# apache/datafusion-comet

Hardware: NVIDIA H100
Metric: rows/sec on TPC-H Q1 filter+agg (higher is better)
Workload: dtype i128

## Files before the change

datafusion-comet_b200/csrc/abi.cpp:

```cpp
#include "../../include/comet_b200.h"

#include "abi_internal.h"
#include "parquet_kernels.h"
#include "exec_internal.h"
#include "jit.h"
#include "plan.h"
#include "proto_wire.h"

#include <cstring>
#include <functional>
#include <map>
#include <mutex>

using namespace cb200;

namespace {

struct CtxRes {
    cudaStream_t stream;
    int* d_err;
    int* h_err;
    cudaEvent_t ev0, ev1;
};
std::mutex g_pool_mu;
std::map<int, std::vector<CtxRes>> g_pool;

void parse_config(const uint8_t* cfg, size_t len, ExecContext& ctx) {
    if (!cfg || !len) return;
    PbReader r(cfg, len);
    while (r.next()) {
        if (r.field != 1 || r.wire != 2) { r.skip(); continue; }
        PbReader e = r.sub();
        std::string k, v;
        while (e.next()) {
            if (e.field == 1) k = e.bytes();
            else if (e.field == 2) v = e.bytes();
            else e.skip();
        }
        if (k == "spark.comet.b200.chunkRows") ctx.chunk_rows = std::max<int64_t>(1024, atoll(v.c_str()));
        else if (k == "spark.comet.batchSize") ctx.batch_size = atoi(v.c_str());
        else if (k == "spark.comet.b200.streamAgg.minRows") ctx.stream_agg_min_rows = atoll(v.c_str());
        else if (k == "spark.comet.b200.streamAgg.maxRatio") ctx.stream_agg_max_ratio = atof(v.c_str());
        else if (k == "spark.comet.b200.hashThreads") { int t = atoi(v.c_str()); if (t == 256 || t == 512 || t == 768 || t == 960) ctx.hash_threads = t; }
    }
}
// ... 5 lines not shown
    cuda_check(cudaSetDevice(ctx.device), "cudaSetDevice");
    {
        struct DevInfo { int major = 0, minor = 0, sms = 0; bool known = false; };
        static DevInfo info[64];
        static std::mutex info_mu;
        std::lock_guard<std::mutex> lk(info_mu);
        if (ctx.device < 0 || ctx.device >= 64) throw ExecError(CB200_ERR_CUDA, "", "device ordinal out of range");
        DevInfo& di = info[ctx.device];
        if (!di.known) {
            cuda_check(cudaDeviceGetAttribute(&di.major, cudaDevAttrComputeCapabilityMajor, ctx.device), "cudaDeviceGetAttribute");
            cuda_check(cudaDeviceGetAttribute(&di.minor, cudaDevAttrComputeCapabilityMinor, ctx.device), "cudaDeviceGetAttribute");
            cuda_check(cudaDeviceGetAttribute(&di.sms, cudaDevAttrMultiProcessorCount, ctx.device), "cudaDeviceGetAttribute");
            di.known = true;
        }
        if (di.major != 9 || di.minor != 0) throw ExecError(CB200_ERR_CUDA, "", "comet_b200 kernels are built for sm_90a; device is sm_" + std::to_string(di.major * 10 + di.minor));
        ctx.num_sms = di.sms;
    }
    {
        std::lock_guard<std::mutex> lk(g_pool_mu);
        auto& fl = g_pool[ctx.device];
        if (!fl.empty()) {
            CtxRes r = fl.back();
            fl.pop_back();
            ctx.stream = r.stream; ctx.d_err = r.d_err; ctx.h_err = r.h_err; ctx.ev0 = r.ev0; ctx.ev1 = r.ev1;
        }
    }
    if (!ctx.stream) {
        cuda_check(cudaStreamCreateWithFlags(&ctx.stream, cudaStreamNonBlocking), "cudaStreamCreate");
        cudaMemPool_t pool;
        if (cudaDeviceGetDefaultMemPool(&pool, ctx.device) == cudaSuccess) {
            unsigned long long keep = ~0ull;
            cudaMemPoolSetAttribute(pool, cudaMemPoolAttrReleaseThreshold, &keep);
        }
        cuda_check(cudaMalloc((void**)&ctx.d_err, 64), "cudaMalloc err");
        cuda_check(cudaMallocHost((void**)&ctx.h_err, 64), "cudaMallocHost err");
        cuda_check(cudaEventCreate(&ctx.ev0), "cudaEventCreate");
        cuda_check(cudaEventCreate(&ctx.ev1), "cudaEventCreate");
    }
    cuda_check(cudaMemsetAsync(ctx.d_err, 0, 64, ctx.stream), "memset err");
    set_alloc_stream(ctx.stream);
    p->root = build_exec(p->op, &ctx, &p->inputs);
    p->started = true;
}

DType dtype_from_ids(int type_id, int precision, int scale) {
    if (type_id < 0 || type_id > 13) throw Unsupported("type id " + std::to_string(type_id));
    DType d;
    d.id = (TypeId)type_id;
    d.precision = precision;
    d.scale = scale;
    return d;
}

}

extern "C" {

const char* cb200_version(void) { return "comet_b200 0.1.0 (sm_90a; reference apache/datafusion-comet 1.1.0 @2699f59b)"; }

int cb200_supports(const uint8_t* op_proto, size_t op_len, cb200_error* why) {
// ... 83 lines not shown
                o.host_values = c.h_data.data();
                o.host_validity_bytes = c.h_valid.empty() ? nullptr : c.h_valid.data();
            } else {
                o.values = c.data ? c.data->ptr : nullptr;
                o.validity = c.validity ? c.validity->ptr : nullptr;
                o.validity_bytes = c.valid_bytes ? c.valid_bytes->ptr : nullptr;
                o.bool_bytes = c.bool_bytes ? c.bool_bytes->ptr : nullptr;
                if (c.is_dict) { o.n_dict = (int)c.dict->values().size(); o.value_width = phys_bytes(c.phys); }
            }
        }
    });
}

void cb200_release(cb200_plan* plan) {
    if (!plan) return;
    TraceSpan ts("release");
    try {
        if (plan->started) cudaSetDevice(plan->ctx.device);
        plan->last = Batch();
        plan->root.reset();
        if (plan->ctx.stream) {
            cudaStreamSynchronize(plan->ctx.stream);
            std::lock_guard<std::mutex> lk(g_pool_mu);
            g_pool[plan->ctx.device].push_back(CtxRes{plan->ctx.stream, plan->ctx.d_err, plan->ctx.h_err, plan->ctx.ev0, plan->ctx.ev1});
        }
        for (auto* s : plan->inputs.streams) if (s && s->release) s->release(s);
    } catch (...) {
    }
    delete plan;
}

cb200_table* cb200_table_create(int64_t n_rows) {
    auto* t = new cb200_table();
    t->t = std::make_shared<DeviceTable>();
    t->t->n_rows = n_rows;
    return t;
}

int cb200_table_add_column(cb200_table* t, int32_t type_id, int32_t precision, int32_t scale, int32_t value_width, const void* dev_values,
                           const void* dev_validity, int64_t null_count, const char* const* dict_values, int32_t n_dict, cb200_error* err) {
    return cb200_guarded(err, [&]() -> int {
        if (!t) throw PlanError("null table handle");
        Column c;
        c.type = dtype_from_ids(type_id, precision, scale);
        size_t n = (size_t)t->t->n_rows;
        if (n_dict > 0) {
            if (!c.type.is_string()) throw PlanError("dictionary values on a non-string column");
// ... 205 lines not shown
```

datafusion-comet_b200/csrc/agg.cpp:

```cpp
#include "exec_internal.h"
#include "../../include/comet_b200.h"

#include "aot_kernels.h"
#include "ranges.h"

#include <algorithm>
#include <mutex>

namespace cb200 {

static std::mutex g_profile_mu;
static std::map<std::string, std::vector<int>> g_range_profile;

void reset_range_profiles() {
    std::lock_guard<std::mutex> lk(g_profile_mu);
    g_range_profile.clear();
}

namespace {

enum class Strategy { Undecided, Dense, Table, Stream };
enum Level { SAFE = 0, TYPE = 1, TIGHT = 2 };
constexpr int DENSE_MAX_GROUPS = 64;

constexpr int GK = CB_GID_RANGES;
struct HashFlags { int w[CB_HFLAG_WORDS]; };
int64_t round_ids(int64_t n) { return (n + GK - 1) / GK * GK; }

using ValueMasks = uint64_t[CB_MAX_COLS * 2];
// ... 2 lines not shown

std::vector<int> decode_gid(int g, const std::vector<int>& cards) {
    std::vector<int> code(cards.size());
    for (int k = (int)cards.size() - 1; k >= 0; k--) { code[(size_t)k] = g % cards[(size_t)k]; g /= cards[(size_t)k]; }
    return code;
}

int grid_for(const ExecContext* ctx, int n_tiles) { return std::max(1, std::min(ctx->num_sms, n_tiles)); }

struct Kernel {
    PipelineSpec spec;
    GeneratedKernel g;
    std::shared_ptr<CompiledModule> mod;
};

void launch_named(ExecContext* ctx, const Kernel& k, const char* name, dim3 grid, dim3 block, void** args) {
    cuda_check(cudaLaunchKernel((const void*)k.mod->kernel(name), grid, block, args, 0, ctx->stream), name);
    ctx->kernel_launches++;
}

struct DenseState {
    std::vector<int> cards;
    std::vector<bool> has_null;
    DeviceBufP totals, spill, partials;
    int groups = 0;

    void regroup(ExecContext* ctx, int n_words, const std::vector<int>& word_kinds, const std::vector<int>& new_cards) {
        int new_groups = 1;
        for (int c : new_cards) new_groups *= c;
        std::vector<uint64_t> oldt((size_t)groups * n_words * 2), newt((size_t)new_groups * n_words * 2);
        cuda_check(cudaMemcpy(oldt.data(), totals->ptr, oldt.size() * 8, cudaMemcpyDeviceToHost), "regroup D2H");
        for (size_t i = 0; i < (size_t)new_groups * n_words; i++) newt[i * 2] = identity_word(word_kinds[i % (size_t)n_words]);
        for (int g = 0; g < groups; g++) {
            const std::vector<int> code = decode_gid(g, cards);
            int ng = 0, mul = 1;
            for (int k = (int)cards.size() - 1; k >= 0; k--) {
                int cd = code[(size_t)k];
                if (has_null[(size_t)k] && cd == cards[(size_t)k] - 1) cd = new_cards[(size_t)k] - 1;
                ng += cd * mul;
                mul *= new_cards[(size_t)k];
            }
            memcpy(&newt[(size_t)ng * n_words * 2], &oldt[(size_t)g * n_words * 2], (size_t)n_words * 16);
        }
        totals = host_to_device(newt.data(), newt.size() * 8, ctx, "regroup H2D");
        groups = new_groups;
    }

// ... 385 lines not shown
    }

    void clear_vmask() {
        if (!vmask) vmask = std::make_shared<DeviceBuf>(CB_MAX_COLS * 16);
        cuda_check(cudaMemsetAsync(vmask->ptr, 0, CB_MAX_COLS * 16, ctx->stream), "memset vmask");
    }
    void copy_vmask(ValueMasks& masks) {
        cuda_check(cudaMemcpyAsync(masks, vmask->ptr, sizeof(ValueMasks), cudaMemcpyDeviceToHost, ctx->stream), "read value masks"); ctx->d2h_bytes += (int64_t)(sizeof(ValueMasks));
    }
    static std::vector<int> mask_bits(const PipelineSpec& spec, const ValueMasks& masks) {
        std::vector<int> seen(spec.cols.size(), -1);
        for (size_t i = 0; i < spec.cols.size(); i++) {
            if (!spec.cols[i].type.is_decimal()) continue;
            uint64_t lo = masks[2 * i], hi = masks[2 * i + 1];
            seen[i] = hi ? 64 + r_bitlen(hi) : r_bitlen(lo);
        }
        return seen;
    }
    void observe(const std::vector<int>& seen) {
        for (size_t i = 0; i < seen.size(); i++)
            if (seen[i] >= 0) observed_bits[(size_t)used_cols[i]] = std::max(observed_bits[(size_t)used_cols[i]], seen[i]);
    }

    int prepare_key(Batch& b, size_t k) {
        int ci = keys[k]->index;
        Column& c = b.cols[ci];
        if (c.type.id == TypeId::Bool) return 2;
        if (!c.type.is_string()) return -1;
        if (c.is_dict) {
            key_dicts[k] = c.dict;
            return (int)c.dict->values().size();
        }
        if (!dev_dicts[k]) {
            auto dd = std::make_shared<DevDict>();
            const int64_t cap = 1 << 16;
            const int max_codes = 4096;
            const int64_t bytes_cap = 1 << 20;
            auto alloc = [&](size_t n) { auto bfr = std::make_shared<DeviceBuf>(n); cuda_check(cudaMemsetAsync(bfr->ptr, 0, bfr->bytes, ctx->stream), "memset dict"); dd->bufs.push_back(bfr); return bfr->ptr; };
            dd->d.tags = (unsigned long long*)alloc((size_t)cap * 8);
            dd->d.slot_code = (int*)alloc((size_t)cap * 4);
            dd->d.capacity = cap;
            dd->d.n_codes = (int*)alloc(64);
            dd->d.bytes_used = (unsigned long long*)((char*)dd->d.n_codes + 16);
            dd->d.err = (int*)((char*)dd->d.n_codes + 32);
            dd->d.max_codes = max_codes;
            dd->d.code_off = (long long*)alloc((size_t)max_codes * 8);
            dd->d.code_len = (int*)alloc((size_t)max_codes * 4);
            dd->d.bytes = (unsigned char*)alloc((size_t)bytes_cap);
            dd->d.bytes_cap = bytes_cap;
            dev_dicts[k] = dd;
            key_dicts[k] = std::make_shared<Dictionary>();
        }
        DevDict& dd = *dev_dicts[k];
        if (!c.offsets || !c.chars) throw Unsupported("string key column without offsets/chars buffers");
        auto row_slot = std::make_shared<DeviceBuf>((size_t)b.n_rows * 4);
        auto codes = std::make_shared<DeviceBuf>((size_t)b.n_rows * 4);
        launch_dict_encode(dd.d, (const int*)c.offsets->ptr, (const unsigned char*)c.chars->ptr, c.validity ? (const unsigned char*)c.validity->ptr : nullptr,
                           b.n_rows, (int*)row_slot->ptr, (int*)codes->ptr, ctx->stream);
        ctx->kernel_launches += 2;
        int hdr[12];
        cuda_check(cudaMemcpyAsync(hdr, dd.d.n_codes, sizeof(hdr), cudaMemcpyDeviceToHost, ctx->stream), "dict header");
        cuda_check(cudaStreamSynchronize(ctx->stream), "dict encode");
        int n_codes = hdr[0], derr = hdr[8];
        if (derr & CB_DICT_FULL) throw Unsupported("plain Utf8 group key with more distinct values than the device dictionary holds (dictionary-encode the column)");
        if (derr & CB_DICT_COLLISION) throw ExecError(14, "", "64-bit hash collision between distinct group key strings");
        if (n_codes > dd.host_known) {
            std::vector<long long> off((size_t)n_codes);
            std::vector<int> len((size_t)n_codes);
            cuda_check(cudaMemcpy(off.data(), dd.d.code_off, (size_t)n_codes * 8, cudaMemcpyDeviceToHost), "dict offsets");
            cuda_check(cudaMemcpy(len.data(), dd.d.code_len, (size_t)n_codes * 4, cudaMemcpyDeviceToHost), "dict lengths");
            for (int i = dd.host_known; i < n_codes; i++) {
                std::string s((size_t)len[(size_t)i], '\0');
                if (len[(size_t)i]) cuda_check(cudaMemcpy(&s[0], dd.d.bytes + off[(size_t)i], (size_t)len[(size_t)i], cudaMemcpyDeviceToHost), "dict bytes");
                key_dicts[k]->append(s);
            }
            dd.host_known = n_codes;
        }
        c.data = codes;
        c.phys = Phys::I32;
        c.is_dict = true;
        c.dict = key_dicts[k];
        return n_codes;
    }

    void consume(Batch& b) {
        for (int ci : used_cols) if (b.cols[(size_t)ci].validity) col_nullable[(size_t)ci] = true;
        std::vector<int> nc(keys.size());
        std::vector<bool> hn(keys.size());
        for (size_t k = 0; k < keys.size(); k++) {
            int card = prepare_key(b, k);
            const Column& c = b.cols[keys[k]->index];
            hn[k] = key_has_null[k] || c.validity != nullptr;
            nc[k] = card < 0 ? -1 : std::max(card, 1) + (hn[k] ? 1 : 0);
            if (!dense.cards.empty() && nc[k] >= 0) nc[k] = std::max(nc[k], dense.cards[k]);
        }
        bool densifiable = true;
        for (int c : nc) if (c < 0) densifiable = false;
// ... 41 lines not shown
            run_range(b, SAMPLE, b.n_rows, n_groups, TIGHT);
        } else {
            run_range(b, 0, b.n_rows, n_groups, have_obs ? TIGHT : TYPE);
        }
        if (!profile_key.empty()) {
            std::lock_guard<std::mutex> lk(g_profile_mu);
            if (g_range_profile.size() > 256) g_range_profile.clear();
            g_range_profile[profile_key] = observed_bits;
        }
    }

    void leave_dense() {
        if (mode == AggMode::Final) throw Unsupported("group cardinality grew past the dense path mid-stream in a Final aggregate");
        if (have_totals()) {
            Batch early;
            dense.finalize(ctx, last, certified_params(), ungrouped, schema, key_dicts, early);
            if (early.n_rows > 0) outq.push_back(std::move(early));
        }
        last = Kernel();
        dense = DenseState();
        n_words = 0; word_kinds.clear(); role_words.clear(); rows_scanned = 0;
    }

    void run_range(Batch& b, int64_t row0, int64_t row1, int n_groups, Level lv) {
        TraceSpan tsr("agg.run_range");
        while (true) {
            Kernel k;
            {
                TraceSpan ts("agg.codegen+jit");
                k = compile(make_spec(&b, Strategy::Dense, n_groups, lv));
            }
            const int64_t max_rows = (int64_t)ctx->num_sms * k.g.threads * (1ll << CB_RPT_LOG2) / 1024 * 1024;
            int64_t r0 = row0;
            while (r0 < row1 && launch_one(b, r0, std::min(row1, r0 + max_rows), n_groups, k, lv)) r0 += max_rows;
            if (r0 >= row1) return;
            if (lv == SAFE) throw ExecError(15, "", "internal: value-mask validation failed without assumptions");
            lv = lv == TIGHT ? TYPE : SAFE;
            row0 = r0;
        }
    }

    bool launch_one(Batch& b, int64_t r0, int64_t r1, int n_groups, const Kernel& k, Level lv) {
        cudaStream_t st = ctx->stream;
        size_t tot_bytes = (size_t)n_groups * n_words * 16;
        if (!have_totals()) {
            dense.totals = std::make_shared<DeviceBuf>(tot_bytes);
            dense.groups = n_groups;
        }
        if (!dense.spill || dense.spill->bytes < tot_bytes) {
            dense.spill = std::make_shared<DeviceBuf>(tot_bytes);
            cuda_check(cudaMemsetAsync(dense.spill->ptr, 0, dense.spill->bytes, st), "memset spill");
        }
        clear_vmask();
        cb::PipeParams p;
        fill_inputs(p, b, k.g.tile, r0, r1);
        bind_str_masks(p, k.spec, b);
        int grid = grid_for(ctx, p.n_tiles);
        size_t part_bytes = (size_t)grid * tot_bytes;
        if (!dense.partials || dense.partials->bytes < part_bytes) dense.partials = std::make_shared<DeviceBuf>(part_bytes);
        p.n_groups = n_groups;
        for (size_t i = 0; i < dense.cards.size() && i < CB_MAX_KEYS; i++) p.key_card[i] = dense.cards[i];
        p.partials = (cb::u8*)dense.partials->ptr;
        p.spill = (cb::u64*)dense.spill->ptr;
        p.vmask = (cb::u64*)vmask->ptr;
        launch(k.mod->kernel(k.g.entry), dim3(grid), dim3(k.g.threads + 32), k.g.dyn_smem(n_groups), &p);
        ctx->pipeline_rows += r1 - r0;
        ValueMasks masks;
        copy_vmask(masks);
        const int errs = ctx->take_device_errors();
        const std::vector<int> seen = mask_bits(k.spec, masks);
        bool ok = true;
        for (size_t i = 0; i < seen.size(); i++)
            if (k.spec.cols[i].assume_bits > 0 && seen[i] > k.spec.cols[i].assume_bits) ok = false;
        observe(seen);
        if (!ok) {
            cuda_check(cudaMemsetAsync(dense.spill->ptr, 0, dense.spill->bytes, st), "memset spill");
            ctx->agg_range_reruns++;
            return false;
        }
        ctx->raise_device_errors(errs);
        ctx->agg_range_levels |= lv == TIGHT ? CB200_RANGE_TIGHT : lv == TYPE ? CB200_RANGE_TYPE : CB200_RANGE_SAFE;
        rows_scanned += r1 - r0;
        cb::FinParams fp;
        memset(&fp, 0, sizeof(fp));
        fp.partials = (const cb::u64*)dense.partials->ptr;
        fp.spill = (cb::u64*)dense.spill->ptr;
        fp.totals = (cb::u64*)dense.totals->ptr;
        fp.n_ctas = grid;
        fp.n_groups = n_groups;
        fp.first = have_totals() ? 0 : 1;
        fp.err = ctx->d_err;
        int total_words = n_groups * n_words;
        void* args[] = {&fp};
        cuda_check(cudaLaunchKernel((const void*)k.mod->kernel("cb_fold"), dim3((total_words + 127) / 128), dim3(128), args, 0, st), "fold launch");
        ctx->kernel_launches++;
        last = k;
        return true;
    }

    void launch_id_rows(Batch& b, int64_t r0, int64_t r1, const Kernel& k, bool with_table) {
        clear_vmask();
        cb::PipeParams p;
        fill_inputs(p, b, k.g.tile, r0, r1);
        bind_str_masks(p, k.spec, b);
        p.hkeys = with_table ? (cb::u64*)table.hkeys->ptr : nullptr;
        p.hkey_of_gid = (cb::u64*)rows.hkey_of_gid->ptr;
        p.htotals = (cb::u64*)rows.htotals->ptr;
        p.hmask = with_table ? (cb::u32)(table.hcap - 1) : 0;
        p.max_groups = (cb::i32)rows.max_groups;
        p.hflags = (cb::i32*)rows.hflags->ptr;
        p.vmask = (cb::u64*)vmask->ptr;
        p.n_groups = 2;
        launch(k.mod->kernel(k.g.entry), dim3(grid_for(ctx, p.n_tiles)), dim3(k.g.threads + 32), k.g.dyn_smem(0), &p);
    }

    void consume_table(Batch& b) {
        const Kernel k = compile(make_spec(&b, Strategy::Table, 2, SAFE));
        {
            TraceSpan ts("hash.ensure_table");
            table.ensure(ctx, k, rows, b.n_rows, child->rows_hint(), rows_scanned, mode != AggMode::Partial || !all_partial);
// ... 88 lines not shown
            fp.cert_b[ai][1] = b >= RSAT ? ~0ull : (uint64_t)(b >> 64);
            const bool direct = aggs[ai].mode != AggMode::Partial || aggs[ai].children[0]->kind == ExprKind::Bound;
            if (b < RSAT && b != 0 && direct) fp.cert_b[ai][1] |= 1ull << 63;
        }
        return fp;
    }

    bool next(Batch& out) override {
        if (!emitted) aggregate_input();
        if (outq_pos >= outq.size()) return false;
        out = std::move(outq[outq_pos++]);
        return true;
    }
    void aggregate_input() {
        if (keys.size() > CB_MAX_KEYS) throw Unsupported("more than 4 group keys");
        key_has_null.assign(keys.size(), false);
        col_nullable.assign(child->schema.size(), false);
        key_dicts.assign(keys.size(), nullptr);
        dev_dicts.assign(keys.size(), nullptr);
        Batch in;
        while (child->next(in)) {
            if (in.n_rows == 0) continue;
            consume(in);
            ctx->check_device_errors();
        }
        emitted = true;
        if (!have_totals()) {
            if (!ungrouped) return;
            last = compile(make_spec(nullptr, Strategy::Dense, 1));
            std::vector<uint64_t> id((size_t)n_words * 2, 0);
            for (int w = 0; w < n_words; w++) id[(size_t)w * 2] = identity_word(word_kinds[(size_t)w]);
            dense.totals = std::make_shared<DeviceBuf>(id.size() * 8);
            cuda_check(cudaMemcpyAsync(dense.totals->ptr, id.data(), id.size() * 8, cudaMemcpyHostToDevice, ctx->stream), "identity totals");
            cuda_check(cudaStreamSynchronize(ctx->stream), "identity totals sync");
            dense.groups = 1;
        }
        Batch result;
        if (strategy == Strategy::Table || strategy == Strategy::Stream) rows.finalize(ctx, last, certified_params(), key_dicts, result);
        else dense.finalize(ctx, last, certified_params(), ungrouped, schema, key_dicts, result);
        outq.push_back(std::move(result));
    }
};

}

ExecNodeP make_agg_node(const OperatorP& agg_op, const ExecNodeP& src, const std::vector<ExprP>& preds, const std::vector<ExprP>& cols, ExecContext* ctx,
                        const std::vector<int>& assume_bits) {
// ... 54 lines not shown
```

datafusion-comet_b200/csrc/exec.cpp:

```cpp
#include "exec_internal.h"

#include <cstdlib>
#include <ctime>
#include <mutex>

namespace cb200 {

enum { ERR_I128_OVERFLOW = 0, ERR_ANSI_OVERFLOW = 1, ERR_ORDER_DEPENDENT = 2, ERR_DIVIDE_BY_ZERO = 3, ERR_ARROW_DIVIDE_BY_ZERO = 4, ERR_DICT_CODE = 5,
       ERR_WIDE_MINMAX = 6 };

bool trace_on() {
    static int on = -1;
    if (on < 0) { const char* e = getenv("CB200_TRACE"); on = (e && *e && *e != '0') ? 1 : 0; }
    return on == 1;
}
double now_ms() {
    struct timespec ts;
    clock_gettime(CLOCK_MONOTONIC, &ts);
    return ts.tv_sec * 1e3 + ts.tv_nsec * 1e-6;
}
TraceSpan::TraceSpan(const char* n) : name(n), t0(trace_on() ? now_ms() : 0) {}
TraceSpan::~TraceSpan() {
    if (trace_on()) { static const double tz = now_ms(); const double t1 = now_ms(); fprintf(stderr, "[cb200 trace] %-28s %8.3f ms   (ends at +%.3f ms)\n", name, t1 - t0, t1 - tz); }
}
// ... 68 lines not shown
        cudaStreamSynchronize(stream);
        e = cudaMallocAsync(&ptr, bytes, stream);
    }
    cuda_check(e, "cudaMallocAsync");
}
DeviceBuf::~DeviceBuf() {
    if (!(owned && ptr)) return;
    if (bytes >= BLOCK_CACHE_MIN && bytes == size_class(bytes)) {
        BlockCache& c = g_block_cache[current_device()];
        cudaEvent_t ev = nullptr;
        if (cudaEventCreateWithFlags(&ev, cudaEventDisableTiming) == cudaSuccess && cudaEventRecord(ev, stream) == cudaSuccess) {
            std::lock_guard<std::mutex> lk(c.mu);
            if (c.cached_bytes + bytes <= block_cache_limit()) {
                c.free_blocks.insert({bytes, CachedBlock{ptr, stream, ev}});
                c.cached_bytes += bytes;
                return;
            }
        }
        if (ev) cudaEventDestroy(ev);
    }
    cudaFreeAsync(ptr, stream);
}

void ExecContext::collect_timing() {
    if (!ev_pending) return;
    float ms = 0;
    if (cudaEventElapsedTime(&ms, ev0, ev1) == cudaSuccess) { pipeline_ms += ms; pipeline_launches++; }
    ev_pending = false;
}

int ExecContext::take_device_errors() {
    cuda_check(cudaMemcpyAsync(h_err, d_err, sizeof(int), cudaMemcpyDeviceToHost, stream), "error flag copy");
    cuda_check(cudaStreamSynchronize(stream), "stream sync");
    collect_timing();
    int e = *h_err;
    if (e) cudaMemsetAsync(d_err, 0, sizeof(int), stream);
    return e;
}

void ExecContext::raise_device_errors(int e) {
    if (!e) return;
    if (e & (1 << ERR_ANSI_OVERFLOW))
        throw ExecError(10, "ARITHMETIC_OVERFLOW", "[ARITHMETIC_OVERFLOW] overflow in ANSI mode");
    if (e & (1 << ERR_DIVIDE_BY_ZERO))
        throw ExecError(10, "DIVIDE_BY_ZERO", "[DIVIDE_BY_ZERO] Division by zero. Use `try_divide` to tolerate divisor being 0 and return NULL instead. "
                                              "If necessary set \"spark.sql.ansi.enabled\" to \"false\" to bypass this error.");
    if (e & (1 << ERR_ARROW_DIVIDE_BY_ZERO)) throw ExecError(11, "", "Arrow error: Divide by zero error");
    if (e & (1 << ERR_I128_OVERFLOW))
        throw ExecError(11, "", "Arrow error: Arithmetic overflow: Overflow happened on decimal arithmetic");
    if (e & (1 << ERR_DICT_CODE))
        throw ExecError(3, "", "dictionary code out of range: a non-NULL row of a dictionary-encoded string column has a code outside its dictionary");
// ... 164 lines not shown
        std::vector<ArrowArray> arrs;
        int64_t total = 0;
        while (total < ctx->chunk_rows) {
            ArrowArray a;
            memset(&a, 0, sizeof(a));
            if (stream->get_next(stream, &a) != 0) {
                const char* m = stream->get_last_error ? stream->get_last_error(stream) : nullptr;
                for (auto& x : arrs) if (x.release) x.release(&x);
                throw ExecError(3, "", std::string("ArrowArrayStream get_next failed: ") + (m ? m : "?"));
            }
            if (!a.release) { eof = true; break; }
            if (a.length > 0) { total += a.length; arrs.push_back(a); }
            else a.release(&a);
        }
        if (arrs.empty()) return false;
        try {
            upload(arrs, total, out);
        } catch (...) {
            for (auto& x : arrs) if (x.release) x.release(&x);
            throw;
        }
        cuda_check(cudaStreamSynchronize(ctx->stream), "H2D copies");
        for (auto& x : arrs) if (x.release) x.release(&x);
        return true;
    }

    std::vector<int32_t> unify_dict(size_t col, const ArrowArray* d) {
        Dictionary& g = *dicts[col];
        const int32_t* off = (const int32_t*)d->buffers[1] + d->offset;
        const char* chars = (const char*)d->buffers[2];
        std::vector<int32_t> remap((size_t)d->length);
        bool identity = true;
        for (int64_t k = 0; k < d->length; k++) {
            const int32_t code = g.intern(std::string(chars + off[k], (size_t)(off[k + 1] - off[k])));
            remap[(size_t)k] = code;
            if (code != k) identity = false;
        }
        if (identity) remap.clear();
        return remap;
    }

    cudaError_t h2d(void* dst, const void* src, size_t n) {
        ctx->h2d_bytes += (int64_t)n;
        return cudaMemcpyAsync(dst, src, n, cudaMemcpyHostToDevice, ctx->stream);
    }

    void upload(std::vector<ArrowArray>& arrs, int64_t total, Batch& out) {
        TraceSpan ts("source.upload");
        out.n_rows = total;
        out.cols.clear();
        out.cols.resize(schema.size());
        cudaStream_t st = ctx->stream;
        for (size_t c = 0; c < schema.size(); c++) {
            Column& col = out.cols[c];
            col.type = schema[c];
            bool any_nulls = false;
            for (auto& a : arrs) {
                ArrowArray* ch = a.children[c];
                if (ch->null_count != 0 && ch->buffers[0]) any_nulls = true;
            }
            if (any_nulls) {
                col.validity = std::make_shared<DeviceBuf>((size_t)(total + 7) / 8 + 8);
                cuda_check(cudaMemsetAsync(col.validity->ptr, 0, col.validity->bytes, st), "memset validity");
            }
            std::vector<DeviceBufP> temps;
            if (col_is_dict[c]) {
                col.is_dict = true;
                col.dict = dicts[c];
                int w = dict_index_width[c];
                bool need_remap = false;
                std::vector<std::vector<int32_t>> remaps;
                for (auto& a : arrs) {
                    remaps.push_back(unify_dict(c, a.children[c]->dictionary));
                    if (!remaps.back().empty()) need_remap = true;
                }
                if (!need_remap) {
                    col.phys = w == 1 ? Phys::I8 : w == 2 ? Phys::I16 : Phys::I32;
                    col.data = std::make_shared<DeviceBuf>((size_t)total * w);
                } else {
                    col.phys = Phys::I32;
                    col.data = std::make_shared<DeviceBuf>((size_t)total * 4);
                }
                int64_t row = 0;
                for (size_t k = 0; k < arrs.size(); k++) {
                    ArrowArray* ch = arrs[k].children[c];
                    const char* src = (const char*)ch->buffers[1] + ch->offset * w;
                    if (!need_remap) {
                        cuda_check(h2d((char*)col.data->ptr + row * w, src, (size_t)ch->length * w), "H2D dict codes");
                    } else {
                        auto tmp = std::make_shared<DeviceBuf>((size_t)ch->length * w);
                        temps.push_back(tmp);
                        cuda_check(h2d(tmp->ptr, src, (size_t)ch->length * w), "H2D dict codes");
                        std::vector<int32_t> table = remaps[k];
                        if (table.empty()) { table.resize((size_t)ch->dictionary->length); for (size_t i = 0; i < table.size(); i++) table[i] = (int32_t)i; }
                        DeviceBufP dt = host_to_device(table.data(), table.size() * 4, ctx, "H2D remap table");
                        ctx->h2d_bytes += (int64_t)(table.size() * 4);
                        temps.push_back(dt);
                        launch_remap_codes(tmp->ptr, w, ch->length, (const int*)dt->ptr, (int)table.size(), (int*)col.data->ptr + row, st);
                    }
                    row += ch->length;
                }
            } else if (schema[c].is_string()) {
                int64_t total_chars = 0;
                for (auto& a : arrs) {
                    ArrowArray* ch = a.children[c];
                    const int32_t* off = (const int32_t*)ch->buffers[1] + ch->offset;
                    total_chars += off[ch->length] - off[0];
                }
                if (total_chars > INT32_MAX) throw Unsupported("more than 2 GiB of string data in one chunk");
                col.chars = std::make_shared<DeviceBuf>((size_t)total_chars + 16);
                std::vector<int32_t> offs((size_t)total + 1);
                int64_t row = 0;
                int32_t base = 0;
                for (auto& a : arrs) {
                    ArrowArray* ch = a.children[c];
                    const int32_t* off = (const int32_t*)ch->buffers[1] + ch->offset;
                    for (int64_t i = 0; i < ch->length; i++) offs[(size_t)(row + i)] = base + (off[i] - off[0]);
                    int32_t nchars = off[ch->length] - off[0];
                    if (nchars) cuda_check(h2d((char*)col.chars->ptr + base, (const char*)ch->buffers[2] + off[0], (size_t)nchars), "H2D chars");
                    base += nchars;
                    row += ch->length;
                }
                offs[(size_t)total] = base;
                col.offsets = host_to_device(offs.data(), offs.size() * 4, ctx, "H2D offsets");
                ctx->h2d_bytes += (int64_t)(offs.size() * 4);
                col.phys = Phys::I32;
            } else {
                col.phys = phys_of(schema[c]);
                int w = schema[c].arrow_width();
                if (w == 0) {
                    col.data = std::make_shared<DeviceBuf>((size_t)(total + 7) / 8 + 8);
                    cuda_check(cudaMemsetAsync(col.data->ptr, 0, col.data->bytes, st), "memset bool");
                    int64_t row = 0;
                    for (auto& a : arrs) {
                        ArrowArray* ch = a.children[c];
                        append_bits((uint32_t*)col.data->ptr, row, (const uint8_t*)ch->buffers[1], ch->offset, ch->length, temps);
                        row += ch->length;
                    }
                } else {
                    col.data = std::make_shared<DeviceBuf>((size_t)total * w);
                    int64_t row = 0;
                    for (auto& a : arrs) {
                        ArrowArray* ch = a.children[c];
                        cuda_check(h2d((char*)col.data->ptr + row * w, (const char*)ch->buffers[1] + ch->offset * w, (size_t)ch->length * w), "H2D column");
                        row += ch->length;
                    }
                }
            }
            if (any_nulls) {
                int64_t row = 0, nulls = 0;
                for (auto& a : arrs) {
                    ArrowArray* ch = a.children[c];
                    bool has = ch->null_count != 0 && ch->buffers[0];
                    append_bits((uint32_t*)col.validity->ptr, row, has ? (const uint8_t*)ch->buffers[0] : nullptr, ch->offset, ch->length, temps);
                    nulls += has ? (ch->null_count < 0 ? 1 : ch->null_count) : 0;
                    row += ch->length;
                }
                col.null_count = nulls;
            }
            if (!temps.empty()) cuda_check(cudaStreamSynchronize(st), "temp buffers");
        }
    }

    void append_bits(uint32_t* dst, int64_t row, const uint8_t* src, int64_t src_off, int64_t n, std::vector<DeviceBufP>& temps) {
        if (n <= 0) return;
        if (src && (row & 7) == 0 && (src_off & 7) == 0 && ((n & 7) == 0)) {
            cuda_check(h2d((char*)dst + (row >> 3), src + (src_off >> 3), (size_t)(n >> 3)), "H2D bitmap");
            return;
        }
        const uint8_t* dsrc = nullptr;
        int64_t doff = 0;
        if (src) {
            int64_t b0 = src_off >> 3, b1 = (src_off + n + 7) >> 3;
            auto tmp = std::make_shared<DeviceBuf>((size_t)(b1 - b0) + 8);
            temps.push_back(tmp);
            cuda_check(h2d(tmp->ptr, src + b0, (size_t)(b1 - b0)), "H2D bitmap");
            dsrc = (const uint8_t*)tmp->ptr;
            doff = src_off & 7;
        }
        launch_bitmap_append(dst, row, dsrc, doff, n, ctx->stream);
    }
};

// ... 459 lines not shown
```

datafusion-comet_b200/csrc/exec.h:

```cpp
#pragma once
#include "arrow_abi.h"
#include "codegen.h"
#include "jit.h"
#include "plan.h"

#include <cuda_runtime.h>
#include <climits>
#include <memory>
#include <string>
#include <unordered_map>
#include <vector>

namespace cb200 {

struct ExecError : std::runtime_error {
    int code;
    std::string error_class;
    ExecError(int c, const std::string& cls, const std::string& msg) : std::runtime_error(msg), code(c), error_class(cls) {}
};

void cuda_check(cudaError_t e, const char* what);

struct TraceSpan {
    const char* name;
// ... 62 lines not shown
    bool on_host = false;
    std::vector<uint8_t> h_data;
    std::vector<uint8_t> h_valid;
    std::vector<int32_t> h_offsets;
};

struct Batch {
    int64_t n_rows = 0;
    std::vector<Column> cols;
};

struct ExecContext {
    int device = 0;
    cudaStream_t stream = nullptr;
    int num_sms = 132;
    int64_t chunk_rows = 1ll << 26;
    int hash_threads = 512;
    int64_t stream_agg_min_rows = 4 << 20;
    double stream_agg_max_ratio = 0.5;
    int batch_size = 8192;
    int* d_err = nullptr;
    int* h_err = nullptr;
    int64_t kernel_launches = 0;
    cudaEvent_t ev0 = nullptr, ev1 = nullptr;
    bool ev_pending = false;
    double pipeline_ms = 0;
    int64_t pipeline_launches = 0;
    int64_t pipeline_rows = 0;
    int64_t h2d_bytes = 0, d2h_bytes = 0;
    int64_t scan_pruned_row_groups = 0, scan_pruned_rows = 0;
    int64_t scan_pruned_pages = 0, scan_page_pruned_rows = 0;
    int64_t agg_strategies = 0;
    int64_t agg_range_levels = 0;
    int64_t agg_range_reruns = 0;
    int64_t sort_rows = 0, sort_passes = 0, sort_pass_rows = 0;
    int64_t sort_select_rows = 0;
    int64_t join_build_rows = 0, join_probe_rows = 0, join_out_rows = 0;
    int64_t join_cond_pairs = 0;
    double partition_ids_ms = 0, partition_place_ms = 0, partition_gather_ms = 0;
    std::vector<int64_t> partition_starts;
    void check_device_errors() { raise_device_errors(take_device_errors()); }
    int take_device_errors();
    void raise_device_errors(int e);
    void collect_timing();
};

struct ExecNode {
    std::vector<DType> schema;
// ... 33 lines not shown
```

datafusion-comet_b200/csrc/exec_internal.h:

```cpp
#pragma once
#include "exec.h"

#include "aot_kernels.h"
#include "device/cb_params.h"

#include <algorithm>
#include <cstring>
#include <functional>
#include <map>
#include <set>

namespace cb200 {

static constexpr size_t SMEM_BUDGET = 220 * 1024;

inline Phys phys_of(const DType& t) {
    switch (t.id) {
    case TypeId::Bool: return Phys::Bitmap;
    case TypeId::Int8: return Phys::I8;
    case TypeId::Int16: return Phys::I16;
    case TypeId::Int32: case TypeId::Date: return Phys::I32;
    case TypeId::Int64: case TypeId::Timestamp: case TypeId::TimestampNtz: return Phys::I64;
    case TypeId::Float32: return Phys::F32;
    case TypeId::Float64: return Phys::F64;
// ... 89 lines not shown
            rewrite_bound(c, slot_of);
            out.push_back(c);
        }
        return out;
    }
    void fill_inputs(cb::PipeParams& p, const Batch& b, int tile, int64_t row0 = 0, int64_t row1 = -1) const { fill_inputs_of(p, b, used_cols, tile, row0, row1); }
    void fill_inputs_of(cb::PipeParams& p, const Batch& b, const std::vector<int>& which, int tile, int64_t row0 = 0, int64_t row1 = -1) const {
        memset(&p, 0, sizeof(p));
        if (row1 < 0) row1 = b.n_rows;
        if (row0 & 1023) throw ExecError(15, "", "internal: launch range must start on a 1024-row boundary");
        for (size_t i = 0; i < which.size(); i++) {
            const Column& c = b.cols[which[i]];
            if (!c.data) throw Unsupported("column " + std::to_string(which[i]) + " (" + c.type.str() + ") has no fixed-width device representation");
            int w = phys_bytes(c.phys);
            p.col[i] = (const cb::u8*)c.data->ptr + (w == 0 ? row0 / 8 : row0 * w);
            p.val[i] = c.validity ? (const cb::u8*)c.validity->ptr + row0 / 8 : nullptr;
        }
        p.n_rows = row1 - row0;
        p.n_tiles = (int)((p.n_rows + tile - 1) / tile);
        p.err = ctx->d_err;
    }
    StrMasks str_masks;
    void bind_str_masks(cb::PipeParams& p, const PipelineSpec& spec, const Batch& b) { str_masks.bind(p, spec, b, ctx); }
    void launch(cudaKernel_t k, dim3 grid, dim3 block, size_t smem, void* params) {
        cuda_check(cudaFuncSetAttribute((const void*)k, cudaFuncAttributeMaxDynamicSharedMemorySize, (int)smem), "cudaFuncSetAttribute(smem)");
        void* args[] = {params};
        if (ctx->ev_pending) { cuda_check(cudaStreamSynchronize(ctx->stream), "stream sync"); ctx->collect_timing(); }
        cuda_check(cudaEventRecord(ctx->ev0, ctx->stream), "event record");
        cuda_check(cudaLaunchKernel((const void*)k, grid, block, args, smem, ctx->stream), "kernel launch");
        cuda_check(cudaEventRecord(ctx->ev1, ctx->stream), "event record");
        ctx->ev_pending = true;
        ctx->kernel_launches++;
    }
};

PipelineSpec count_pass_spec(std::vector<SourceCol> cols, std::vector<ExprP> predicates);

ExecNodeP make_agg_node(const OperatorP& agg_op, const ExecNodeP& src, const std::vector<ExprP>& preds, const std::vector<ExprP>& cols, ExecContext* ctx,
                        const std::vector<int>& assume_bits);
ExecNodeP make_partition_node(const OperatorP& op, const ExecNodeP& child, ExecContext* ctx);
ExecNodeP make_sort_node(const OperatorP& op, const ExecNodeP& child, ExecContext* ctx);
ExecNodeP make_join_node(const OperatorP& op, const ExecNodeP& left, const ExecNodeP& right, ExecContext* ctx);

int key_kind(const Column& c);
DeviceBufP host_to_device(const void* p, size_t n, ExecContext* ctx, const char* what);
void columns_to_device(Batch& b, ExecContext* ctx);
void arrive(Batch& b, ExecContext* ctx, const char* op);
Batch drain(ExecNode& child, ExecContext* ctx, const char* op, const char* concat_op);
template <typename I> void gather_columns(const Batch& in, const I* row_idx, int64_t n, Batch& out, ExecContext* ctx, const char* op);
void gather_columns_or_null(const Batch& in, const unsigned* row_idx, int64_t n, Batch& out, ExecContext* ctx);
Batch concat_batches(const std::vector<Batch>& bs, ExecContext* ctx, const char* op);
cb::SortKeyCol key_field(const Column& c, bool has_null, int& off);
struct RowKeys { DeviceBufP keys; uint64_t and_or[2 * cb::SK_MAX_WORDS]; std::vector<int> digits; };
RowKeys pack_row_keys(const cb::SortKeyCols& kc, int64_t n, int bits, ExecContext* ctx);
// ... 10 lines not shown
```

Before: 38.87 billion.

## Batch dense-agg sub-range launches and defer host syncs and validation readback

The dense aggregation path now launches all sub-range pipeline kernels back to back, each with its own partials/spill slot and value-mask scratch, then does a single D2H readback and stream sync before validating and folding. Previously every sub-range did its own launch, vmask copy and sync. Several other syncs go too: the per-column temp-buffer sync during upload (host vectors are kept alive until the batch sync instead), the per-batch device error check, and the per-string copies when decoding the string dictionary, which now uses one prefetch copy. Timing events become a growable per-launch array. The cost is more device memory for per-slot buffers, plus more complex rerun logic that recurses into fresh slots.

```diff
diff --git a/datafusion-comet_b200/csrc/abi.cpp b/datafusion-comet_b200/csrc/abi.cpp
--- a/datafusion-comet_b200/csrc/abi.cpp
+++ b/datafusion-comet_b200/csrc/abi.cpp
@@ -20,7 +20,7 @@
     cudaStream_t stream;
     int* d_err;
     int* h_err;
-    cudaEvent_t ev0, ev1;
+    std::vector<cudaEvent_t> ev;
 };
 std::mutex g_pool_mu;
 std::map<int, std::vector<CtxRes>> g_pool;
@@ -72,7 +72,7 @@
         if (!fl.empty()) {
             CtxRes r = fl.back();
             fl.pop_back();
-            ctx.stream = r.stream; ctx.d_err = r.d_err; ctx.h_err = r.h_err; ctx.ev0 = r.ev0; ctx.ev1 = r.ev1;
+            ctx.stream = r.stream; ctx.d_err = r.d_err; ctx.h_err = r.h_err; ctx.ev = r.ev;
         }
     }
     if (!ctx.stream) {
@@ -84,8 +84,6 @@
         }
         cuda_check(cudaMalloc((void**)&ctx.d_err, 64), "cudaMalloc err");
         cuda_check(cudaMallocHost((void**)&ctx.h_err, 64), "cudaMallocHost err");
-        cuda_check(cudaEventCreate(&ctx.ev0), "cudaEventCreate");
-        cuda_check(cudaEventCreate(&ctx.ev1), "cudaEventCreate");
     }
     cuda_check(cudaMemsetAsync(ctx.d_err, 0, 64, ctx.stream), "memset err");
     set_alloc_stream(ctx.stream);
@@ -215,7 +213,7 @@
         if (plan->ctx.stream) {
             cudaStreamSynchronize(plan->ctx.stream);
             std::lock_guard<std::mutex> lk(g_pool_mu);
-            g_pool[plan->ctx.device].push_back(CtxRes{plan->ctx.stream, plan->ctx.d_err, plan->ctx.h_err, plan->ctx.ev0, plan->ctx.ev1});
+            g_pool[plan->ctx.device].push_back(CtxRes{plan->ctx.stream, plan->ctx.d_err, plan->ctx.h_err, plan->ctx.ev});
         }
         for (auto* s : plan->inputs.streams) if (s && s->release) s->release(s);
     } catch (...) {
diff --git a/datafusion-comet_b200/csrc/agg.cpp b/datafusion-comet_b200/csrc/agg.cpp
--- a/datafusion-comet_b200/csrc/agg.cpp
+++ b/datafusion-comet_b200/csrc/agg.cpp
@@ -5,6 +5,7 @@
 #include "ranges.h"
 
 #include <algorithm>
+#include <climits>
 #include <mutex>
 
 namespace cb200 {
@@ -53,7 +54,7 @@
 struct DenseState {
     std::vector<int> cards;
     std::vector<bool> has_null;
-    DeviceBufP totals, spill, partials;
+    DeviceBufP totals;
     int groups = 0;
 
     void regroup(ExecContext* ctx, int n_words, const std::vector<int>& word_kinds, const std::vector<int>& new_cards) {
@@ -485,6 +486,7 @@
             if (seen[i] >= 0) observed_bits[(size_t)used_cols[i]] = std::max(observed_bits[(size_t)used_cols[i]], seen[i]);
     }
 
+    static constexpr size_t DICT_PREFETCH = 1 << 16;
     int prepare_key(Batch& b, size_t k) {
         int ci = keys[k]->index;
         Column& c = b.cols[ci];
@@ -499,7 +501,14 @@
             const int64_t cap = 1 << 16;
             const int max_codes = 4096;
             const int64_t bytes_cap = 1 << 20;
-            auto alloc = [&](size_t n) { auto bfr = std::make_shared<DeviceBuf>(n); cuda_check(cudaMemsetAsync(bfr->ptr, 0, bfr->bytes, ctx->stream), "memset dict"); dd->bufs.push_back(bfr); return bfr->ptr; };
+            const size_t sizes[] = {(size_t)cap * 8, (size_t)cap * 4, 64, (size_t)max_codes * 8, (size_t)max_codes * 4, (size_t)bytes_cap};
+            size_t total = 0;
+            for (size_t s : sizes) total += (s + 255) / 256 * 256;
+            auto whole = std::make_shared<DeviceBuf>(total);
+            cuda_check(cudaMemsetAsync(whole->ptr, 0, whole->bytes, ctx->stream), "memset dict");
+            dd->bufs.push_back(whole);
+            size_t at = 0;
+            auto alloc = [&](size_t n) { void* q = (char*)whole->ptr + at; at += (n + 255) / 256 * 256; return q; };
             dd->d.tags = (unsigned long long*)alloc((size_t)cap * 8);
             dd->d.slot_code = (int*)alloc((size_t)cap * 4);
             dd->d.capacity = cap;
@@ -521,21 +530,31 @@
         launch_dict_encode(dd.d, (const int*)c.offsets->ptr, (const unsigned char*)c.chars->ptr, c.validity ? (const unsigned char*)c.validity->ptr : nullptr,
                            b.n_rows, (int*)row_slot->ptr, (int*)codes->ptr, ctx->stream);
         ctx->kernel_launches += 2;
+        const char* head = (const char*)dd.d.n_codes;
+        const size_t o_off = (size_t)((const char*)dd.d.code_off - head), o_len = (size_t)((const char*)dd.d.code_len - head);
+        const size_t o_bytes = (size_t)((const char*)dd.d.bytes - head);
+        std::unique_ptr<char[]> h(new char[o_bytes + DICT_PREFETCH]);
+        cuda_check(cudaMemcpyAsync(h.get(), head, o_bytes + DICT_PREFETCH, cudaMemcpyDeviceToHost, ctx->stream), "dict header");
+        cuda_check(cudaStreamSynchronize(ctx->stream), "dict encode");
         int hdr[12];
-        cuda_check(cudaMemcpyAsync(hdr, dd.d.n_codes, sizeof(hdr), cudaMemcpyDeviceToHost, ctx->stream), "dict header");
-        cuda_check(cudaStreamSynchronize(ctx->stream), "dict encode");
+        memcpy(hdr, h.get(), sizeof(hdr));
         int n_codes = hdr[0], derr = hdr[8];
         if (derr & CB_DICT_FULL) throw Unsupported("plain Utf8 group key with more distinct values than the device dictionary holds (dictionary-encode the column)");
         if (derr & CB_DICT_COLLISION) throw ExecError(14, "", "64-bit hash collision between distinct group key strings");
         if (n_codes > dd.host_known) {
-            std::vector<long long> off((size_t)n_codes);
-            std::vector<int> len((size_t)n_codes);
-            cuda_check(cudaMemcpy(off.data(), dd.d.code_off, (size_t)n_codes * 8, cudaMemcpyDeviceToHost), "dict offsets");
-            cuda_check(cudaMemcpy(len.data(), dd.d.code_len, (size_t)n_codes * 4, cudaMemcpyDeviceToHost), "dict lengths");
+            const long long* off = (const long long*)(h.get() + o_off);
+            const int* len = (const int*)(h.get() + o_len);
+            long long lo = LLONG_MAX, hi = 0;
+            for (int i = dd.host_known; i < n_codes; i++) { lo = std::min(lo, off[i]); hi = std::max(hi, off[i] + len[i]); }
+            const char* bytes = h.get() + o_bytes;
+            std::vector<char> more;
+            if (hi > (long long)DICT_PREFETCH) {
+                more.resize((size_t)(hi - lo));
+                cuda_check(cudaMemcpy(more.data(), dd.d.bytes + lo, more.size(), cudaMemcpyDeviceToHost), "dict bytes");
+            }
             for (int i = dd.host_known; i < n_codes; i++) {
-                std::string s((size_t)len[(size_t)i], '\0');
-                if (len[(size_t)i]) cuda_check(cudaMemcpy(&s[0], dd.d.bytes + off[(size_t)i], (size_t)len[(size_t)i], cudaMemcpyDeviceToHost), "dict bytes");
-                key_dicts[k]->append(s);
+                const char* sp = more.empty() ? bytes + off[i] : more.data() + (off[i] - lo);
+                key_dicts[k]->append(std::string(sp, (size_t)len[i]));
             }
             dd.host_known = n_codes;
         }
@@ -623,80 +642,96 @@
         n_words = 0; word_kinds.clear(); role_words.clear(); rows_scanned = 0;
     }
 
-    void run_range(Batch& b, int64_t row0, int64_t row1, int n_groups, Level lv) {
+    void run_range(Batch& b, int64_t row0, int64_t row1, int n_groups, Level lv, size_t slot0 = 0) {
         TraceSpan tsr("agg.run_range");
-        while (true) {
-            Kernel k;
-            {
-                TraceSpan ts("agg.codegen+jit");
-                k = compile(make_spec(&b, Strategy::Dense, n_groups, lv));
-            }
-            const int64_t max_rows = (int64_t)ctx->num_sms * k.g.threads * (1ll << CB_RPT_LOG2) / 1024 * 1024;
-            int64_t r0 = row0;
-            while (r0 < row1 && launch_one(b, r0, std::min(row1, r0 + max_rows), n_groups, k, lv)) r0 += max_rows;
-            if (r0 >= row1) return;
-            if (lv == SAFE) throw ExecError(15, "", "internal: value-mask validation failed without assumptions");
-            lv = lv == TIGHT ? TYPE : SAFE;
-            row0 = r0;
-        }
-    }
-
-    bool launch_one(Batch& b, int64_t r0, int64_t r1, int n_groups, const Kernel& k, Level lv) {
-        cudaStream_t st = ctx->stream;
-        size_t tot_bytes = (size_t)n_groups * n_words * 16;
+        Kernel k;
+        {
+            TraceSpan ts("agg.codegen+jit");
+            k = compile(make_spec(&b, Strategy::Dense, n_groups, lv));
+        }
+        const int64_t max_rows = (int64_t)ctx->num_sms * k.g.threads * (1ll << CB_RPT_LOG2) / 1024 * 1024;
+        const size_t tot_bytes = (size_t)n_groups * n_words * 16;
         if (!have_totals()) {
             dense.totals = std::make_shared<DeviceBuf>(tot_bytes);
             dense.groups = n_groups;
         }
-        if (!dense.spill || dense.spill->bytes < tot_bytes) {
-            dense.spill = std::make_shared<DeviceBuf>(tot_bytes);
-            cuda_check(cudaMemsetAsync(dense.spill->ptr, 0, dense.spill->bytes, st), "memset spill");
-        }
-        clear_vmask();
-        cb::PipeParams p;
-        fill_inputs(p, b, k.g.tile, r0, r1);
-        bind_str_masks(p, k.spec, b);
-        int grid = grid_for(ctx, p.n_tiles);
-        size_t part_bytes = (size_t)grid * tot_bytes;
-        if (!dense.partials || dense.partials->bytes < part_bytes) dense.partials = std::make_shared<DeviceBuf>(part_bytes);
-        p.n_groups = n_groups;
-        for (size_t i = 0; i < dense.cards.size() && i < CB_MAX_KEYS; i++) p.key_card[i] = dense.cards[i];
-        p.partials = (cb::u8*)dense.partials->ptr;
-        p.spill = (cb::u64*)dense.spill->ptr;
-        p.vmask = (cb::u64*)vmask->ptr;
-        launch(k.mod->kernel(k.g.entry), dim3(grid), dim3(k.g.threads + 32), k.g.dyn_smem(n_groups), &p);
-        ctx->pipeline_rows += r1 - r0;
-        ValueMasks masks;
-        copy_vmask(masks);
-        const int errs = ctx->take_device_errors();
-        const std::vector<int> seen = mask_bits(k.spec, masks);
-        bool ok = true;
-        for (size_t i = 0; i < seen.size(); i++)
-            if (k.spec.cols[i].assume_bits > 0 && seen[i] > k.spec.cols[i].assume_bits) ok = false;
-        observe(seen);
-        if (!ok) {
-            cuda_check(cudaMemsetAsync(dense.spill->ptr, 0, dense.spill->bytes, st), "memset spill");
-            ctx->agg_range_reruns++;
-            return false;
-        }
-        ctx->raise_device_errors(errs);
-        ctx->agg_range_levels |= lv == TIGHT ? CB200_RANGE_TIGHT : lv == TYPE ? CB200_RANGE_TYPE : CB200_RANGE_SAFE;
-        rows_scanned += r1 - r0;
-        cb::FinParams fp;
-        memset(&fp, 0, sizeof(fp));
-        fp.partials = (const cb::u64*)dense.partials->ptr;
-        fp.spill = (cb::u64*)dense.spill->ptr;
-        fp.totals = (cb::u64*)dense.totals->ptr;
-        fp.n_ctas = grid;
-        fp.n_groups = n_groups;
-        fp.first = have_totals() ? 0 : 1;
-        fp.err = ctx->d_err;
-        int total_words = n_groups * n_words;
-        void* args[] = {&fp};
-        cuda_check(cudaLaunchKernel((const void*)k.mod->kernel("cb_fold"), dim3((total_words + 127) / 128), dim3(128), args, 0, st), "fold launch");
-        ctx->kernel_launches++;
-        last = k;
-        return true;
+        const size_t n_sub = (size_t)((row1 - row0 + max_rows - 1) / max_rows);
+        ensure_slots(slot0 + n_sub, tot_bytes);
+        cudaStream_t st = ctx->stream;
+        cuda_check(cudaMemsetAsync((char*)sub_scratch->ptr + slot0 * SUB_SCRATCH, 0, n_sub * SUB_SCRATCH, st), "memset value masks");
+        std::vector<int> grids(n_sub);
+        for (size_t j = 0; j < n_sub; j++) {
+            const int64_t r0 = row0 + (int64_t)j * max_rows, r1 = std::min(row1, r0 + max_rows);
+            SubSlot& s = slots[slot0 + j];
+            cb::PipeParams p;
+            fill_inputs(p, b, k.g.tile, r0, r1);
+            bind_str_masks(p, k.spec, b);
+            grids[j] = grid_for(ctx, p.n_tiles);
+            if (!s.partials || s.partials->bytes < (size_t)grids[j] * tot_bytes) s.partials = std::make_shared<DeviceBuf>((size_t)grids[j] * tot_bytes);
+            p.n_groups = n_groups;
+            for (size_t i = 0; i < dense.cards.size() && i < CB_MAX_KEYS; i++) p.key_card[i] = dense.cards[i];
+            p.partials = (cb::u8*)s.partials->ptr;
+            p.spill = (cb::u64*)s.spill->ptr;
+            p.vmask = (cb::u64*)((char*)sub_scratch->ptr + (slot0 + j) * SUB_SCRATCH);
+            p.err = (int*)((char*)p.vmask + sizeof(ValueMasks));
+            launch(k.mod->kernel(k.g.entry), dim3(grids[j]), dim3(k.g.threads + 32), k.g.dyn_smem(n_groups), &p, (int)j);
+            ctx->pipeline_rows += r1 - r0;
+        }
+        std::vector<uint8_t> h((size_t)n_sub * SUB_SCRATCH);
+        cuda_check(cudaMemcpyAsync(h.data(), (char*)sub_scratch->ptr + slot0 * SUB_SCRATCH, h.size(), cudaMemcpyDeviceToHost, st), "read value masks");
+        ctx->d2h_bytes += (int64_t)h.size();
+        cuda_check(cudaStreamSynchronize(st), "stream sync");
+        ctx->collect_timing();
+        std::vector<bool> ok(n_sub, true);
+        for (size_t j = 0; j < n_sub; j++) {
+            const std::vector<int> seen = mask_bits(k.spec, *(const ValueMasks*)(h.data() + j * SUB_SCRATCH));
+            for (size_t i = 0; i < seen.size(); i++)
+                if (k.spec.cols[i].assume_bits > 0 && seen[i] > k.spec.cols[i].assume_bits) ok[j] = false;
+            observe(seen);
+        }
+        for (size_t j = 0; j < n_sub; j++) {
+            const int64_t r0 = row0 + (int64_t)j * max_rows, r1 = std::min(row1, r0 + max_rows);
+            SubSlot& s = slots[slot0 + j];
+            const bool same_layout = k.g.n_words == n_words && k.g.word_kinds == word_kinds && k.g.role_words == role_words;
+            if (!ok[j] || !same_layout) {
+                cuda_check(cudaMemsetAsync(s.spill->ptr, 0, s.spill->bytes, st), "memset spill");
+                ctx->agg_range_reruns++;
+                if (lv == SAFE) throw ExecError(15, "", "internal: value-mask validation failed without assumptions");
+                run_range(b, r0, r1, n_groups, lv == TIGHT ? TYPE : SAFE, slot0 + n_sub);
+                continue;
+            }
+            ctx->raise_device_errors(*(const int*)(h.data() + j * SUB_SCRATCH + sizeof(ValueMasks)));
+            ctx->agg_range_levels |= lv == TIGHT ? CB200_RANGE_TIGHT : lv == TYPE ? CB200_RANGE_TYPE : CB200_RANGE_SAFE;
+            rows_scanned += r1 - r0;
+            cb::FinParams fp;
+            memset(&fp, 0, sizeof(fp));
+            fp.partials = (const cb::u64*)s.partials->ptr;
+            fp.spill = (cb::u64*)s.spill->ptr;
+            fp.totals = (cb::u64*)dense.totals->ptr;
+            fp.n_ctas = grids[j];
+            fp.n_groups = n_groups;
+            fp.first = have_totals() ? 0 : 1;
+            fp.err = ctx->d_err;
+            int total_words = n_groups * n_words;
+            void* args[] = {&fp};
+            cuda_check(cudaLaunchKernel((const void*)k.mod->kernel("cb_fold"), dim3((total_words + 127) / 128), dim3(128), args, 0, st), "fold launch");
+            ctx->kernel_launches++;
+            last = k;
+        }
+    }
+
+    struct SubSlot { DeviceBufP partials, spill; };
+    static constexpr size_t SUB_SCRATCH = sizeof(ValueMasks) + 16;
+    std::vector<SubSlot> slots;
+    DeviceBufP sub_scratch;
+    void ensure_slots(size_t n, size_t tot_bytes) {
+        if (slots.size() < n) slots.resize(n);
+        for (SubSlot& s : slots) {
+            if (s.spill && s.spill->bytes >= tot_bytes) continue;
+            s.spill = std::make_shared<DeviceBuf>(tot_bytes);
+            cuda_check(cudaMemsetAsync(s.spill->ptr, 0, s.spill->bytes, ctx->stream), "memset spill");
+        }
+        if (!sub_scratch || sub_scratch->bytes < n * SUB_SCRATCH) sub_scratch = std::make_shared<DeviceBuf>(n * SUB_SCRATCH);
     }
 
     void launch_id_rows(Batch& b, int64_t r0, int64_t r1, const Kernel& k, bool with_table) {
@@ -831,7 +866,6 @@
         while (child->next(in)) {
             if (in.n_rows == 0) continue;
             consume(in);
-            ctx->check_device_errors();
         }
         emitted = true;
         if (!have_totals()) {
diff --git a/datafusion-comet_b200/csrc/exec.cpp b/datafusion-comet_b200/csrc/exec.cpp
--- a/datafusion-comet_b200/csrc/exec.cpp
+++ b/datafusion-comet_b200/csrc/exec.cpp
@@ -114,11 +114,22 @@
     cudaFreeAsync(ptr, stream);
 }
 
+void ExecContext::record_timing(int pair, bool end) {
+    while (ev.size() < 2 * (size_t)pair + 2) {
+        cudaEvent_t e;
+        cuda_check(cudaEventCreate(&e), "cudaEventCreate");
+        ev.push_back(e);
+    }
+    cuda_check(cudaEventRecord(ev[2 * (size_t)pair + (end ? 1 : 0)], stream), "event record");
+    if (end) ev_pending = std::max(ev_pending, pair + 1);
+}
+
 void ExecContext::collect_timing() {
-    if (!ev_pending) return;
-    float ms = 0;
-    if (cudaEventElapsedTime(&ms, ev0, ev1) == cudaSuccess) { pipeline_ms += ms; pipeline_launches++; }
-    ev_pending = false;
+    for (int i = 0; i < ev_pending; i++) {
+        float ms = 0;
+        if (cudaEventElapsedTime(&ms, ev[2 * (size_t)i], ev[2 * (size_t)i + 1]) == cudaSuccess) { pipeline_ms += ms; pipeline_launches++; }
+    }
+    ev_pending = 0;
 }
 
 int ExecContext::take_device_errors() {
@@ -329,6 +340,7 @@
         }
         cuda_check(cudaStreamSynchronize(ctx->stream), "H2D copies");
         for (auto& x : arrs) if (x.release) x.release(&x);
+        host_staged.clear();
         return true;
     }
 
@@ -351,6 +363,14 @@
         ctx->h2d_bytes += (int64_t)n;
         return cudaMemcpyAsync(dst, src, n, cudaMemcpyHostToDevice, ctx->stream);
     }
+    std::vector<std::vector<int32_t>> host_staged;
+    DeviceBufP stage_h2d(std::vector<int32_t> v, const char* what) {
+        auto d = std::make_shared<DeviceBuf>(v.size() * 4);
+        host_staged.push_back(std::move(v));
+        const std::vector<int32_t>& h = host_staged.back();
+        if (!h.empty()) cuda_check(h2d(d->ptr, h.data(), h.size() * 4), what);
+        return d;
+    }
 
     void upload(std::vector<ArrowArray>& arrs, int64_t total, Batch& out) {
         TraceSpan ts("source.upload");
@@ -358,6 +378,7 @@
         out.cols.clear();
         out.cols.resize(schema.size());
         cudaStream_t st = ctx->stream;
+        std::vector<DeviceBufP> temps;
         for (size_t c = 0; c < schema.size(); c++) {
             Column& col = out.cols[c];
             col.type = schema[c];
@@ -370,7 +391,6 @@
                 col.validity = std::make_shared<DeviceBuf>((size_t)(total + 7) / 8 + 8);
                 cuda_check(cudaMemsetAsync(col.validity->ptr, 0, col.validity->bytes, st), "memset validity");
             }
-            std::vector<DeviceBufP> temps;
             if (col_is_dict[c]) {
                 col.is_dict = true;
                 col.dict = dicts[c];
@@ -400,10 +420,10 @@
                         cuda_check(h2d(tmp->ptr, src, (size_t)ch->length * w), "H2D dict codes");
                         std::vector<int32_t> table = remaps[k];
                         if (table.empty()) { table.resize((size_t)ch->dictionary->length); for (size_t i = 0; i < table.size(); i++) table[i] = (int32_t)i; }
-                        DeviceBufP dt = host_to_device(table.data(), table.size() * 4, ctx, "H2D remap table");
-                        ctx->h2d_bytes += (int64_t)(table.size() * 4);
+                        const int n_table = (int)table.size();
+                        DeviceBufP dt = stage_h2d(std::move(table), "H2D remap table");
                         temps.push_back(dt);
-                        launch_remap_codes(tmp->ptr, w, ch->length, (const int*)dt->ptr, (int)table.size(), (int*)col.data->ptr + row, st);
+                        launch_remap_codes(tmp->ptr, w, ch->length, (const int*)dt->ptr, n_table, (int*)col.data->ptr + row, st);
                     }
                     row += ch->length;
                 }
@@ -429,8 +449,7 @@
                     row += ch->length;
                 }
                 offs[(size_t)total] = base;
-                col.offsets = host_to_device(offs.data(), offs.size() * 4, ctx, "H2D offsets");
-                ctx->h2d_bytes += (int64_t)(offs.size() * 4);
+                col.offsets = stage_h2d(std::move(offs), "H2D offsets");
                 col.phys = Phys::I32;
             } else {
                 col.phys = phys_of(schema[c]);
@@ -465,7 +484,6 @@
                 }
                 col.null_count = nulls;
             }
-            if (!temps.empty()) cuda_check(cudaStreamSynchronize(st), "temp buffers");
         }
     }
 
diff --git a/datafusion-comet_b200/csrc/exec.h b/datafusion-comet_b200/csrc/exec.h
--- a/datafusion-comet_b200/csrc/exec.h
+++ b/datafusion-comet_b200/csrc/exec.h
@@ -108,8 +108,9 @@
     int* d_err = nullptr;
     int* h_err = nullptr;
     int64_t kernel_launches = 0;
-    cudaEvent_t ev0 = nullptr, ev1 = nullptr;
-    bool ev_pending = false;
+    std::vector<cudaEvent_t> ev;
+    int ev_pending = 0;
+    void record_timing(int pair, bool end);
     double pipeline_ms = 0;
     int64_t pipeline_launches = 0;
     int64_t pipeline_rows = 0;
diff --git a/datafusion-comet_b200/csrc/exec_internal.h b/datafusion-comet_b200/csrc/exec_internal.h
--- a/datafusion-comet_b200/csrc/exec_internal.h
+++ b/datafusion-comet_b200/csrc/exec_internal.h
@@ -135,14 +135,14 @@
     }
     StrMasks str_masks;
     void bind_str_masks(cb::PipeParams& p, const PipelineSpec& spec, const Batch& b) { str_masks.bind(p, spec, b, ctx); }
-    void launch(cudaKernel_t k, dim3 grid, dim3 block, size_t smem, void* params) {
+    void launch(cudaKernel_t k, dim3 grid, dim3 block, size_t smem, void* params, int pair = 0) {
         cuda_check(cudaFuncSetAttribute((const void*)k, cudaFuncAttributeMaxDynamicSharedMemorySize, (int)smem), "cudaFuncSetAttribute(smem)");
         void* args[] = {params};
-        if (ctx->ev_pending) { cuda_check(cudaStreamSynchronize(ctx->stream), "stream sync"); ctx->collect_timing(); }
-        cuda_check(cudaEventRecord(ctx->ev0, ctx->stream), "event record");
+        if (pair == 0 && ctx->ev_pending) { cuda_check(cudaStreamSynchronize(ctx->stream), "stream sync"); ctx->collect_timing(); }
+        if (pair != ctx->ev_pending) throw ExecError(15, "", "internal: pipeline timing events out of order");
+        ctx->record_timing(pair, false);
         cuda_check(cudaLaunchKernel((const void*)k, grid, block, args, smem, ctx->stream), "kernel launch");
-        cuda_check(cudaEventRecord(ctx->ev1, ctx->stream), "event record");
-        ctx->ev_pending = true;
+        ctx->record_timing(pair, true);
         ctx->kernel_launches++;
     }
 };
```

Measured after the change: 39.42 billion, median of 6. Within noise of the previous version (+1.4%).
